# beautifulv0id/Convex-2D-GPU-Collision-Detection

Hardware: AMD Instinct MI355X
Metric: sat_pair_tests_per_s (higher is better)
Workload: dtype f32

## Files before the change

### convex-2d-gpu-collision-detection_amd/csrc/c2d_poly.hip

```cpp
#include "c2d_internal.hpp"
#include "c2d_math.hpp"
#include "c2d_count.hpp"
#include "c2d_wave.hpp"

namespace c2d {

constexpr int kSlots = 8;

template <int KM, int MIN_WAVES, bool FULL>
__global__ __launch_bounds__(64, MIN_WAVES) void sat_poly_kernel(const float* __restrict__ vx, const float* __restrict__ vy,
                                                                 const uint8_t* __restrict__ kcnt, size_t n, int rows_arg,
                                                                 uint8_t* __restrict__ out,
                                                                 unsigned long long* __restrict__ d_count,
                                                                 CountWs words,
                                                                 uint32_t* __restrict__ async_err)
{
    const int rows = FULL ? KM : rows_arg;
    constexpr int LP = 2 * KM;
    constexpr int PP = 64 / LP;
    __shared__ __attribute__((aligned(16))) float2 s_slot[kSlots][2 * KM];
    const uint32_t lane = threadIdx.x;
    uint32_t n_collide = 0;
    const size_t n_tiles = (n + 63) / 64;
    for (size_t tile = blockIdx.x; tile < n_tiles; tile += gridDim.x) {
        const size_t p0 = tile * 64;
        const uint32_t here = (uint32_t)((n - p0) < (size_t)64 ? (n - p0) : (size_t)64);
        const bool in = lane < here;
        const uint32_t cl = in ? lane : here - 1;
        int ka = kcnt[p0 + cl], kb = kcnt[n + p0 + cl];
        const bool bad = ka < 1 || ka > rows || kb < 1 || kb > rows;
        ka = ka < 1 ? 1 : (ka > rows ? rows : ka);
        kb = kb < 1 ? 1 : (kb > rows ? rows : kb);
        if (__ballot(bad) != 0 && lane == 0) __hip_atomic_fetch_or(async_err, 1u, __ATOMIC_RELAXED, __HIP_MEMORY_SCOPE_SYSTEM);
        const int kmaxA = (int)wave_max_u32((uint32_t)ka), kmaxB = (int)wave_max_u32((uint32_t)kb);
        float ax[KM], ay[KM], bx[KM], by[KM];
        const float* rx = vx + p0;
        const float* ry = vy + p0;
        uint32_t off = cl * 4u;
        auto ld = [&off](const float* row) {
            asm volatile("" : "+v"(off));
            return __builtin_nontemporal_load(reinterpret_cast<const float*>(reinterpret_cast<const char*>(row) + off));
        };
#pragma unroll
        for (int r = 0; r < KM; r++) {
            if (r < kmaxA) {
                ax[r] = ld(rx);
                ay[r] = ld(ry);
            } else {
                ax[r] = 0.0f;
                ay[r] = 0.0f;
            }
            rx += n;
            ry += n;
        }
        if constexpr (!FULL) {
            rx = vx + (size_t)rows * n + p0;
            ry = vy + (size_t)rows * n + p0;
        }
#pragma unroll
        for (int r = 0; r < KM; r++) {
            if (r < kmaxB) {
                bx[r] = ld(rx);
                by[r] = ld(ry);
            } else {
                bx[r] = 0.0f;
                by[r] = 0.0f;
            }
            rx += n;
            ry += n;
        }
        float sax = ax[0], say = ay[0], sbx = bx[0], sby = by[0];
#pragma unroll
        for (int r = 1; r < KM; r++) {
            const bool ua = r < ka, ub = r < kb;
            ax[r] = ua ? ax[r] : ax[0];
            ay[r] = ua ? ay[r] : ay[0];
            bx[r] = ub ? bx[r] : bx[0];
            by[r] = ub ? by[r] : by[0];
            if (r < kmaxA) { sax += ax[r]; say += ay[r]; }
            if (r < kmaxB) { sbx += bx[r]; sby += by[r]; }
        }
        const float fka = (float)ka, fkb = (float)kb;
        const float ia = __builtin_amdgcn_rcpf(fka), ib = __builtin_amdgcn_rcpf(fkb);
        float dX = (sbx - (float)(kmaxB - kb) * bx[0]) * ib - (sax - (float)(kmaxA - ka) * ax[0]) * ia;
        float dY = (sby - (float)(kmaxB - kb) * by[0]) * ib - (say - (float)(kmaxA - ka) * ay[0]) * ia;
        {
            const float c = (ax[1] - ax[0]) * (ay[2] - ay[0]) - (ay[1] - ay[0]) * (ax[2] - ax[0]);
            const uint32_t sgn = __float_as_uint(c) & 0x80000000u;
            dX = __uint_as_float(__float_as_uint(dX) ^ sgn);
            dY = __uint_as_float(__float_as_uint(dY) ^ sgn);
        }
        float best = -__builtin_inff(), nx1 = 0.0f, ny1 = 0.0f;
#pragma unroll
        for (int r = 0; r < KM; r++) {
            if (r < kmaxA) {
                const int r1 = (r + 1) & (KM - 1);
                const float ey = ay[r1] - ay[r];
                const float nx = -ey;
                const float ny = ax[r1] - ax[r];
                const float nd = fma_(nx, dX, ny * dY);
                const float l2 = fma_(nx, nx, ny * ny);
                const float s = nd * __builtin_amdgcn_rsqf(l2);
                const bool better = s > best;
                best = better ? s : best;
                nx1 = better ? nx : nx1;
                ny1 = better ? ny : ny1;
            }
        }
        float mnA = __builtin_inff(), mxA = -__builtin_inff(), mnB = __builtin_inff(), mxB = -__builtin_inff();
#pragma unroll
        for (int r = 0; r < KM; r++)
            if (r < kmaxA) poly_minmax(nx1, ny1, ax[r], ay[r], mnA, mxA);
#pragma unroll
        for (int r = 0; r < KM; r++)
            if (r < kmaxB) poly_minmax(nx1, ny1, bx[r], by[r], mnB, mxB);
        bool sep = ((mxA < mnB) || (mxB < mnA)) && first_projections_ordered(nx1 * ax[0] + ny1 * ay[0], nx1 * bx[0] + ny1 * by[0]);
        sep = sep || bad;
        unsigned long long todo = __ballot(in && !sep);
        while (todo) {
            uint32_t lane2 = lane;
            asm volatile("" : "+v"(lane2));
            const int a = (int)(lane2 % LP);
            const int sub = (int)(lane2 / LP);
            const int i0 = a, i1 = (a & KM) | ((a + 1) & (KM - 1));
            const uint32_t rank = __builtin_amdgcn_mbcnt_hi((uint32_t)(todo >> 32), __builtin_amdgcn_mbcnt_lo((uint32_t)todo, 0u));
            const bool park = ((todo >> lane) & 1ull) && rank < (uint32_t)kSlots;
            __syncthreads();
            if (park) {
                float4* S4 = reinterpret_cast<float4*>(&s_slot[rank][0]);
#pragma unroll
                for (int r = 0; r < KM / 2; r++) {
                    S4[r] = make_float4(ax[2 * r], ay[2 * r], ax[2 * r + 1], ay[2 * r + 1]);
                    S4[KM / 2 + r] = make_float4(bx[2 * r], by[2 * r], bx[2 * r + 1], by[2 * r + 1]);
                }
            }
            __syncthreads();
            const int left = __popcll(todo);
            const int g = left < kSlots ? left : kSlots;
            for (int i = 0; i < g; i += PP) {
                const int cnt = (g - i) < PP ? (g - i) : PP;
                int j[PP];
                int kA = 0, kB = 0;
#pragma unroll
                for (int q = 0; q < PP; q++) {
                    j[q] = -1;
                    if (q < cnt) {
                        j[q] = __ffsll((long long)todo) - 1;
                        todo &= todo - 1;
                        const int kaq = __builtin_amdgcn_readlane(ka, j[q]), kbq = __builtin_amdgcn_readlane(kb, j[q]);
                        kA = kaq > kA ? kaq : kA;
                        kB = kbq > kB ? kbq : kB;
                    }
                }
                const float2* S = &s_slot[i + (sub < cnt ? sub : 0)][0];
                const float4* S4 = reinterpret_cast<const float4*>(S);
                const float2 e0 = S[i0], e1 = S[i1];
                const float nx = -(e1.y - e0.y), ny = e1.x - e0.x;
                float mn1 = __builtin_inff(), mx1 = -__builtin_inff(), mn2 = __builtin_inff(), mx2 = -__builtin_inff();
                float4 q4 = S4[0];
                for (int r2 = 0; 2 * r2 < kA; r2++) {
                    const float4 qn = S4[r2 + 1];
                    poly_minmax(nx, ny, q4.x, q4.y, mn1, mx1);
                    poly_minmax(nx, ny, q4.z, q4.w, mn1, mx1);
                    q4 = qn;
                }
                q4 = S4[KM / 2];
                for (int r2 = 0; 2 * r2 < kB; r2++) {
                    const float4 qn = S4[KM / 2 + ((r2 + 1) & (KM / 2 - 1))];
                    poly_minmax(nx, ny, q4.x, q4.y, mn2, mx2);
                    poly_minmax(nx, ny, q4.z, q4.w, mn2, mx2);
                    q4 = qn;
                }
                const float pa0 = nx * S[0].x + ny * S[0].y, pb0 = nx * S[KM].x + ny * S[KM].y;
                const unsigned long long bal = __ballot(((mx1 < mn2) || (mx2 < mn1)) && first_projections_ordered(pa0, pb0));
                constexpr unsigned long long kPairMask = LP == 64 ? ~0ull : ((1ull << LP) - 1ull);
#pragma unroll
                for (int q = 0; q < PP; q++) {
                    const bool any = ((bal >> (q * LP)) & kPairMask) != 0ull;
                    sep = ((int)lane == j[q]) ? any : sep;
                }
            }
        }
        const bool collide = in && !sep;
        if (in) out[p0 + lane] = collide ? (uint8_t)1 : (uint8_t)0;
        n_collide += (uint32_t)__popcll(__ballot(collide));
    }
    if (d_count) wave_count_arrive_total2(n_collide, d_count, words);
}


__global__ __launch_bounds__(64) void sat_poly4_kernel(const float* __restrict__ vx, const float* __restrict__ vy,
                                                       const uint8_t* __restrict__ kcnt, size_t n, size_t n_groups,
                                                       uint8_t* __restrict__ out, unsigned long long* __restrict__ d_count,
                                                       CountWs words, uint32_t* __restrict__ async_err)
{
    uint32_t my_count = 0;
    bool any_bad = false;
    const size_t stride = (size_t)gridDim.x * 64;
    for (size_t g = (size_t)blockIdx.x * 64 + threadIdx.x; g < n_groups; g += stride) {
        f32x4 X[8], Y[8];
#pragma unroll
        for (int r = 0; r < 8; r++) {
            X[r] = __builtin_nontemporal_load(reinterpret_cast<const f32x4*>(vx + (size_t)r * n) + g);
            Y[r] = __builtin_nontemporal_load(reinterpret_cast<const f32x4*>(vy + (size_t)r * n) + g);
        }
        const uint32_t kA4 = __builtin_nontemporal_load(reinterpret_cast<const uint32_t*>(kcnt) + g);
        const uint32_t kB4 = __builtin_nontemporal_load(reinterpret_cast<const uint32_t*>(kcnt + n) + g);
        uint32_t packed = 0;
#pragma unroll
        for (int e = 0; e < 4; e++) {
            int ka = (int)((kA4 >> (8 * e)) & 0xffu), kb = (int)((kB4 >> (8 * e)) & 0xffu);
            const bool bad = ka < 1 || ka > 4 || kb < 1 || kb > 4;
            any_bad |= bad;
            ka = ka < 1 ? 1 : (ka > 4 ? 4 : ka);
            kb = kb < 1 ? 1 : (kb > 4 ? 4 : kb);
            float px[8], py[8];
#pragma unroll
            for (int r = 0; r < 4; r++) {
                px[r] = r < ka ? X[r][e] : X[0][e];
                py[r] = r < ka ? Y[r][e] : Y[0][e];
                px[4 + r] = r < kb ? X[4 + r][e] : X[4][e];
                py[4 + r] = r < kb ? Y[4 + r][e] : Y[4][e];
            }
            bool sep = false;
#pragma unroll
            for (int a = 0; a < 8; a++) {
                const int i0 = a, i1 = (a & 4) | ((a + 1) & 3);
                const float nx = -(py[i1] - py[i0]), ny = px[i1] - px[i0];
                float mn1 = __builtin_inff(), mx1 = -__builtin_inff(), mn2 = __builtin_inff(), mx2 = -__builtin_inff();
#pragma unroll
                for (int r = 0; r < 4; r++) {
                    poly_minmax(nx, ny, px[r], py[r], mn1, mx1);
                    poly_minmax(nx, ny, px[4 + r], py[4 + r], mn2, mx2);
                }
                sep |= ((mx1 < mn2) || (mx2 < mn1)) && first_projections_ordered(nx * px[0] + ny * py[0], nx * px[4] + ny * py[4]);
            }
            packed |= ((sep || bad) ? 0u : 1u) << (8 * e);
        }
        my_count += (uint32_t)__popc(packed);
        __builtin_nontemporal_store(packed, reinterpret_cast<uint32_t*>(out) + g);
    }
    if (__ballot(any_bad) != 0 && threadIdx.x == 0) __hip_atomic_fetch_or(async_err, 1u, __ATOMIC_RELAXED, __HIP_MEMORY_SCOPE_SYSTEM);
    if (d_count) wave_count_arrive(my_count, d_count, words);
}

int launch_poly_onebin(c2d_ctx* ctx, hipStream_t s, const float* d_vx, const float* d_vy, const uint8_t* d_k, size_t n, int rows, uint8_t* d_out,
                       unsigned long long* d_count, uint32_t* async_err);

template <int KM, int MIN_WAVES, bool FULL>
static void launch_poly(c2d_ctx* ctx, hipStream_t s, const float* d_vx, const float* d_vy, const uint8_t* d_k, size_t n, int rows, uint8_t* d_out,
                        unsigned long long* d_count, uint32_t* async_err)
{
#ifndef C2D_POLY_PADDED_TILES_PER_WAVE
#define C2D_POLY_PADDED_TILES_PER_WAVE 1
#endif
    const size_t n_tiles = (n + 63) / 64;
    const size_t want = (n_tiles + C2D_POLY_PADDED_TILES_PER_WAVE - 1) / C2D_POLY_PADDED_TILES_PER_WAVE;
    const int grid = (int)(want < (size_t)kMaxGrid ? want : (size_t)kMaxGrid);
    hipLaunchKernelGGL((sat_poly_kernel<KM, MIN_WAVES, FULL>), dim3(grid), dim3(64), 0, s, d_vx, d_vy, d_k, n, rows, d_out, d_count,
                       workspace_count_ticket2(ctx, s, (size_t)grid, d_count != nullptr), async_err);
}

}

using namespace c2d;

extern "C" {

int c2d_sat_poly_pairs_rows(c2d_ctx* ctx, const float* d_vx, const float* d_vy, const uint8_t* d_k, size_t n, int rows,
                            uint8_t* d_out, unsigned long long* d_count, c2d_stream stream)
{
    if (!ctx) return C2D_ERR_INVALID_ARG;
    if (rows < 1 || rows > C2D_POLY_KMAX) return fail_arg(ctx, "c2d_sat_poly_pairs_rows: rows must be 1..C2D_POLY_KMAX");
    if (n == 0) return C2D_OK;
    if (!d_vx || !d_vy || !d_k || !d_out) return fail_arg(ctx, "c2d_sat_poly_pairs: NULL argument");
    DeviceGuard g(ctx->device);
    hipStream_t s = (hipStream_t)stream;
    if (int rc = workspace_acquire(ctx, s, d_count != nullptr)) return rc;
    uint32_t* err = ctx->d_async_err;
    auto aligned = [](const void* p, size_t a) { return (reinterpret_cast<uintptr_t>(p) & (a - 1)) == 0; };
    if (rows == 4 && n % 4 == 0 && aligned(d_vx, 16) && aligned(d_vy, 16) && aligned(d_k, 4) && aligned(d_out, 4)) {
        const size_t n_groups = n / 4;
        const size_t blocks = (n_groups + 63) / 64;
        const size_t grid = blocks < (size_t)kMaxGrid ? blocks : (size_t)kMaxGrid;
        hipLaunchKernelGGL(sat_poly4_kernel, dim3((unsigned)grid), dim3(64), 0, s, d_vx, d_vy, d_k, n, n_groups, d_out, d_count,
                           workspace_count_ticket(ctx, s, grid, d_count != nullptr), err);
    } else if (rows == 16) launch_poly<16, 5, true>(ctx, s, d_vx, d_vy, d_k, n, rows, d_out, d_count, err);
    else if (rows > 8) {
        if (launch_poly_onebin(ctx, s, d_vx, d_vy, d_k, n, rows, d_out, d_count, err) != C2D_OK)
            launch_poly<16, 5, false>(ctx, s, d_vx, d_vy, d_k, n, rows, d_out, d_count, err);
    }
    else if (rows > 4) launch_poly<8, 7, false>(ctx, s, d_vx, d_vy, d_k, n, rows, d_out, d_count, err);
    else launch_poly<4, 8, false>(ctx, s, d_vx, d_vy, d_k, n, rows, d_out, d_count, err);
    C2D_LAUNCH_CHECK(ctx);
    return C2D_OK;
}

int c2d_sat_poly_pairs(c2d_ctx* ctx, const float* d_vx, const float* d_vy, const uint8_t* d_k, size_t n, uint8_t* d_out,
                       unsigned long long* d_count, c2d_stream stream)
{
    return c2d_sat_poly_pairs_rows(ctx, d_vx, d_vy, d_k, n, C2D_POLY_KMAX, d_out, d_count, stream);
}

}
```

Baseline: 98.29 billion.

## Pack variable-size polygon pairs into wave lanes by actual edge count

```diff
diff --git a/convex-2d-gpu-collision-detection_amd/csrc/c2d_poly.hip b/convex-2d-gpu-collision-detection_amd/csrc/c2d_poly.hip
--- a/convex-2d-gpu-collision-detection_amd/csrc/c2d_poly.hip
+++ b/convex-2d-gpu-collision-detection_amd/csrc/c2d_poly.hip
@@ -5,7 +5,20 @@
 
 namespace c2d {
 
-constexpr int kSlots = 8;
+constexpr int kSlots = 12;
+constexpr int kTripPairs = 8;
+
+C2D_DEV uint32_t wave_max_dpp(uint32_t v)
+{
+    auto mx = [](uint32_t a, int b) { return a > (uint32_t)b ? a : (uint32_t)b; };
+    v = mx(v, __builtin_amdgcn_update_dpp(0, (int)v, 0x111, 0xf, 0xf, true));
+    v = mx(v, __builtin_amdgcn_update_dpp(0, (int)v, 0x112, 0xf, 0xf, true));
+    v = mx(v, __builtin_amdgcn_update_dpp(0, (int)v, 0x114, 0xf, 0xf, true));
+    v = mx(v, __builtin_amdgcn_update_dpp(0, (int)v, 0x118, 0xf, 0xf, true));
+    v = mx(v, __builtin_amdgcn_update_dpp((int)v, (int)v, 0x142, 0xa, 0xf, false));
+    v = mx(v, __builtin_amdgcn_update_dpp((int)v, (int)v, 0x143, 0xc, 0xf, false));
+    return (uint32_t)__builtin_amdgcn_readlane((int)v, 63);
+}
 
 template <int KM, int MIN_WAVES, bool FULL>
 __global__ __launch_bounds__(64, MIN_WAVES) void sat_poly_kernel(const float* __restrict__ vx, const float* __restrict__ vy,
@@ -16,9 +29,8 @@
                                                                  uint32_t* __restrict__ async_err)
 {
     const int rows = FULL ? KM : rows_arg;
-    constexpr int LP = 2 * KM;
-    constexpr int PP = 64 / LP;
-    __shared__ __attribute__((aligned(16))) float2 s_slot[kSlots][2 * KM];
+    __shared__ __attribute__((aligned(16))) float2 s_slot[kSlots][2 * KM + 2];
+    __shared__ uint32_t s_size[16];
     const uint32_t lane = threadIdx.x;
     uint32_t n_collide = 0;
     const size_t n_tiles = (n + 63) / 64;
@@ -32,7 +44,7 @@
         ka = ka < 1 ? 1 : (ka > rows ? rows : ka);
         kb = kb < 1 ? 1 : (kb > rows ? rows : kb);
         if (__ballot(bad) != 0 && lane == 0) __hip_atomic_fetch_or(async_err, 1u, __ATOMIC_RELAXED, __HIP_MEMORY_SCOPE_SYSTEM);
-        const int kmaxA = (int)wave_max_u32((uint32_t)ka), kmaxB = (int)wave_max_u32((uint32_t)kb);
+        const int kmaxA = (int)wave_max_dpp((uint32_t)ka), kmaxB = (int)wave_max_dpp((uint32_t)kb);
         float ax[KM], ay[KM], bx[KM], by[KM];
         const float* rx = vx + p0;
         const float* ry = vy + p0;
@@ -117,12 +129,10 @@
         bool sep = ((mxA < mnB) || (mxB < mnA)) && first_projections_ordered(nx1 * ax[0] + ny1 * ay[0], nx1 * bx[0] + ny1 * by[0]);
         sep = sep || bad;
         unsigned long long todo = __ballot(in && !sep);
+        unsigned long long sepmask = 0;
         while (todo) {
             uint32_t lane2 = lane;
             asm volatile("" : "+v"(lane2));
-            const int a = (int)(lane2 % LP);
-            const int sub = (int)(lane2 / LP);
-            const int i0 = a, i1 = (a & KM) | ((a + 1) & (KM - 1));
             const uint32_t rank = __builtin_amdgcn_mbcnt_hi((uint32_t)(todo >> 32), __builtin_amdgcn_mbcnt_lo((uint32_t)todo, 0u));
             const bool park = ((todo >> lane) & 1ull) && rank < (uint32_t)kSlots;
             __syncthreads();
@@ -133,26 +143,45 @@
                     S4[r] = make_float4(ax[2 * r], ay[2 * r], ax[2 * r + 1], ay[2 * r + 1]);
                     S4[KM / 2 + r] = make_float4(bx[2 * r], by[2 * r], bx[2 * r + 1], by[2 * r + 1]);
                 }
+                s_size[rank] = ((uint32_t)ka << 5) | (uint32_t)kb;
             }
             __syncthreads();
             const int left = __popcll(todo);
             const int g = left < kSlots ? left : kSlots;
-            for (int i = 0; i < g; i += PP) {
-                const int cnt = (g - i) < PP ? (g - i) : PP;
-                int j[PP];
+            const bool has = lane2 < (uint32_t)g;
+            const uint32_t size = s_size[lane2 & 15u];
+            const int lp = has ? (int)((size >> 5) + (size & 31u)) : 0;
+            int pinc = lp;
+            pinc += __builtin_amdgcn_update_dpp(0, pinc, 0x111, 0xf, 0xf, true);
+            pinc += __builtin_amdgcn_update_dpp(0, pinc, 0x112, 0xf, 0xf, true);
+            pinc += __builtin_amdgcn_update_dpp(0, pinc, 0x114, 0xf, 0xf, true);
+            pinc += __builtin_amdgcn_update_dpp(0, pinc, 0x118, 0xf, 0xf, true);
+            const int pex = pinc - lp;
+            const uint32_t word = ((uint32_t)pex << 14) | ((lane2 & 15u) << 10) | size;
+            int i = 0, base = 0;
+            uint32_t sepq = 0;
+            while (i < g) {
+                const bool member = has && (lane2 - (uint32_t)i) < (uint32_t)kTripPairs && pinc - base <= 64;
+                const int cnt = __popcll(__ballot(member));
+                if (cnt < kTripPairs && i + cnt == g && i > 0 && left > g) break;
+                const uint32_t key = ((lane2 + (uint32_t)base) << 14) | 0x3fffu;
+                uint32_t w = 0;
                 int kA = 0, kB = 0;
-#pragma unroll
-                for (int q = 0; q < PP; q++) {
-                    j[q] = -1;
-                    if (q < cnt) {
-                        j[q] = __ffsll((long long)todo) - 1;
-                        todo &= todo - 1;
-                        const int kaq = __builtin_amdgcn_readlane(ka, j[q]), kbq = __builtin_amdgcn_readlane(kb, j[q]);
-                        kA = kaq > kA ? kaq : kA;
-                        kB = kbq > kB ? kbq : kB;
-                    }
-                }
-                const float2* S = &s_slot[i + (sub < cnt ? sub : 0)][0];
+                for (int q = 0; q < cnt; q++) {
+                    const uint32_t wq = (uint32_t)__builtin_amdgcn_readlane((int)word, i + q);
+                    w = wq <= key ? wq : w;
+                    const int kaq = (int)((wq >> 5) & 31u), kbq = (int)(wq & 31u);
+                    kA = kaq > kA ? kaq : kA;
+                    kB = kbq > kB ? kbq : kB;
+                }
+                const int a = (int)(lane2 + (uint32_t)base) - (int)(w >> 14);
+                const int kal = (int)((w >> 5) & 31u), kbl = (int)(w & 31u);
+                const bool edge_of_a = a < kal;
+                const int en = edge_of_a ? kal : kbl, eb = edge_of_a ? 0 : KM;
+                int ei = edge_of_a ? a : a - kal;
+                ei = ei < en - 1 ? ei : en - 1;
+                const int i0 = eb + ei, i1 = eb + (ei + 1 == en ? 0 : ei + 1);
+                const float2* S = &s_slot[(w >> 10) & 15u][0];
                 const float4* S4 = reinterpret_cast<const float4*>(S);
                 const float2 e0 = S[i0], e1 = S[i1];
                 const float nx = -(e1.y - e0.y), ny = e1.x - e0.x;
@@ -173,16 +202,20 @@
                 }
                 const float pa0 = nx * S[0].x + ny * S[0].y, pb0 = nx * S[KM].x + ny * S[KM].y;
                 const unsigned long long bal = __ballot(((mx1 < mn2) || (mx2 < mn1)) && first_projections_ordered(pa0, pb0));
-                constexpr unsigned long long kPairMask = LP == 64 ? ~0ull : ((1ull << LP) - 1ull);
-#pragma unroll
-                for (int q = 0; q < PP; q++) {
-                    const bool any = ((bal >> (q * LP)) & kPairMask) != 0ull;
-                    sep = ((int)lane == j[q]) ? any : sep;
-                }
-            }
-        }
+                const uint32_t slice = (uint32_t)(bal >> (((word >> 14) - (uint32_t)base) & 63u)) << ((32u - ((word >> 5) & 31u) - (word & 31u)) & 31u);
+                sepq |= (uint32_t)__ballot(member && slice != 0u);
+                base = __builtin_amdgcn_readlane(pinc, i + cnt - 1);
+                i += cnt;
+            }
+            const bool done = park && rank < (uint32_t)i;
+            sepmask |= __ballot(done && ((sepq >> rank) & 1u) != 0u);
+            todo &= ~__ballot(done);
+        }
+        uint32_t lane3 = lane;
+        asm volatile("" : "+v"(lane3));
+        sep = sep || ((sepmask >> lane3) & 1ull) != 0ull;
         const bool collide = in && !sep;
-        if (in) out[p0 + lane] = collide ? (uint8_t)1 : (uint8_t)0;
+        if (in) out[p0 + lane3] = collide ? (uint8_t)1 : (uint8_t)0;
         n_collide += (uint32_t)__popcll(__ballot(collide));
     }
     if (d_count) wave_count_arrive_total2(n_collide, d_count, words);
```

Result: slower. 94.14 billion (-4.2%).
